# waldstein94/Stratified-Transformer

Hardware: AMD Instinct MI355X
Metric: points/sec through StratifiedAttention fwd+bwd, 100k-pt scene (higher is better)
Workload: dtype f32

## Files before the change

### include/pointops2_hip.h

```cpp
#ifndef POINTOPS2_HIP_H
#define POINTOPS2_HIP_H

#include <stddef.h>
#include <stdint.h>

#ifdef __cplusplus
extern "C" {
#endif

void pointops2_set_stream(void *hip_stream);
void *pointops2_get_stream(void);
const char *pointops2_last_error(void);
int pointops2_abi_version(void);
void pointops2_diag_set_fps_patience(unsigned long long ticks_100mhz);


void furthestsampling_cuda_launcher(int b, int n, const float *xyz, const int *offset,
                                    const int *new_offset, float *tmp, int *idx);

void knnquery_cuda_launcher(int m, int nsample, const float *xyz, const float *new_xyz,
                            const int *offset, const int *new_offset, int *idx, float *dist2);

void grouping_forward_cuda_launcher(int m, int nsample, int c, const float *input, const int *idx, float *output);
void grouping_backward_cuda_launcher(int m, int nsample, int c, const float *grad_output, const int *idx, float *grad_input);
// ... 144 lines not shown
    int n_pairs;
    int n_keyslots;
    const int *counts;
    const int *parent_first;
    const int *cell_perm;
    const int *cell_qstart;
    const int *cell_kbase;
    const int *cell_pbase;
    const int *cell_order;
    const int *qcell;
    const int *cell_keys;
    const int *kcell;
    const unsigned int *relp;
    int task_first;
    int task_step;
    int table_rows;
    int max_queries;
    const int *task_list;
    const int *task_count;
} pointops2_cell_plan;
size_t pointops2_cell_plan_workspace_bytes(int N);
void pointops2_cell_plan_count_launcher(int N, int max_queries, const int *s_cluster, const int *s_starts, const int *l_cluster,
                                        const int *ls_starts, int *cell_order, int *qcell, int *cell_desc, int *cell_qstart,
                                        int *cell_kbase, int *cell_pbase, int *cell_perm, int *parent_first, int *counts, void *ws,
                                        size_t ws_bytes);
void pointops2_cell_plan_prepare_launcher(int N, int max_queries, const int *s_cluster, const int *l_cluster, int *cell_order,
                                          int *parent_first, int *counts, void *ws, size_t ws_bytes);
void pointops2_cell_plan_sizes_launcher(int N, const int *s_cluster, const int *s_starts, const int *l_cluster, const int *ls_starts,
                                        const int *cell_order, int *qcell, int *cell_desc, int *cell_qstart, int *cell_kbase,
                                        int *cell_pbase, int *cell_perm, int *counts, void *ws, size_t ws_bytes);
void pointops2_cell_plan_fill_launcher(int N, const float *xyz, float window, float quant, int L, const int *s_order, const int *ls,
                                       const float *wc, const int *cell_order, const int *qcell, const int *cell_qstart,
                                       const int *cell_desc, const int *cell_kbase, const int *cell_pbase, int *cell_keys, int *kcell,
                                       unsigned int *relp);
void pointops2_swin_quant_launcher(int N, const float *xyz, const float *bbox6, float window, float quant, int shifted, int *q);
void pointops2_swin_pairs_rel_launcher(int N, int M, const int *index_0, const int *index_1, const int *q, int qgl, int *rel_idx);
void pointops2_swin_cell_fill_launcher(int N, int L, int qgl, const int *q, const int *s_order, const int *ls, const float *wc,
                                       const int *cell_order, const int *qcell, const int *cell_qstart, const int *cell_desc,
                                       const int *cell_kbase, const int *cell_pbase, int *cell_keys, int *kcell, unsigned int *relp);
void cell_attention_forward_launcher(const pointops2_cell_plan *plan, int h, int hdim, int L, const float *q, const float *k,
                                     const float *v, const float *table_q, const float *table_k, const float *table_v, float *out,
                                     float *ml, float *pbuf);
void cell_attention_backward_launcher(const pointops2_cell_plan *plan, int h, int hdim, int L, const float *grad_out, const float *q,
                                      const float *k, const float *v, const float *out, const float *table_q, const float *table_k,
                                      const float *table_v, const float *pbuf, float *gsbuf, float *grad_q, float *grad_k,
                                      float *grad_v, float *grad_table_q, float *grad_table_k, float *grad_table_v);
#define POINTOPS2_CELL_FWD_ERROR   (-1)
#define POINTOPS2_CELL_FWD_NONE    0
#define POINTOPS2_CELL_FWD_MFMA64  1
#define POINTOPS2_CELL_FWD_MFMA80  2
#define POINTOPS2_CELL_FWD_VALU80  3
#define POINTOPS2_CELL_FWD_VALU160 4
int pointops2_cell_forward_variant(const pointops2_cell_plan *plan, int h, int hdim, int L, int bf16);

void pointops2_voxel_keys_launcher(int N, int is_f64, const void *coord, double voxel, unsigned long long *keys);
void pointops2_crop_dist_launcher(int N, int is_f64, const void *coord, int seed, void *dist);

void cell_attention_forward_bf16_launcher(const pointops2_cell_plan *plan, int h, int hdim, int L, const uint16_t *q, const uint16_t *k,
                                          const uint16_t *v, const uint16_t *table_q, const uint16_t *table_k, const uint16_t *table_v,
                                          float *out, float *ml, float *pbuf);
void cell_attention_backward_bf16_launcher(const pointops2_cell_plan *plan, int h, int hdim, int L, const float *grad_out, const uint16_t *q,
                                           const uint16_t *k, const uint16_t *v, const float *out, const uint16_t *table_q,
                                           const uint16_t *table_k, const uint16_t *table_v, const float *pbuf, float *gsbuf, float *grad_q,
                                           float *grad_k, float *grad_v, float *grad_table_q, float *grad_table_k, float *grad_table_v);
#define POINTOPS2_ROWS_F32  0
#define POINTOPS2_ROWS_F16  1
#define POINTOPS2_ROWS_BF16 2
void cell_attention_qkv_forward_launcher(const pointops2_cell_plan *plan, int h, int hdim, int L, const void *qkv, int row_type, float scale,
                                         const float *table_q, const float *table_k, const float *table_v, float *out, float *ml, float *pbuf);
void cell_attention_qkv_backward_launcher(const pointops2_cell_plan *plan, int h, int hdim, int L, const float *grad_out, const void *qkv, int row_type,
                                          float scale, const float *out, const float *table_q, const float *table_k, const float *table_v,
                                          const float *pbuf, float *gsbuf, float *grad_qkv, float *grad_table_q, float *grad_table_k,
                                          float *grad_table_v);

void kpconv_aggregate_forward_launcher(int n_q, int n_s, int n_nb, int c, int n_kp, const float *query_xyz, const float *support_xyz,
                                       const int *neighbors, const float *feat, const float *k_points, float extent, float *wf);
void kpconv_aggregate_backward_launcher(int n_q, int n_s, int n_nb, int c, int n_kp, const float *query_xyz, const float *support_xyz,
                                        const int *neighbors, const float *k_points, float extent, const float *grad_wf,
                                        float *grad_feat);

void grouped_max_forward_launcher(int m, int n_s, int k, int c, int row_type, const void *feat, const int *idx, void *out,
                                  unsigned char *arg);
void grouped_max_backward_launcher(int m, int n_s, int k, int c, int row_type, const void *grad_out, const unsigned char *arg,
                                   const int *src_offsets, const int *src_pair, void *grad_feat);

void residual_norm_forward_launcher(int n, int c, int y_type, int o_type, const float *x, const void *y, const float *s, const float *gamma,
                                    const float *beta, float eps, float *z, void *o, float *stat);
void residual_norm_backward_launcher(int n, int c, int y_type, int o_type, const void *grad_o, const float *grad_z, const float *z,
                                     const float *stat, const float *s, const float *gamma, float *grad_x, void *grad_y, float *partials,
                                     int partial_rows, float *grad_gamma, float *grad_beta);

#define POINTOPS2_ACT_NONE       0
#define POINTOPS2_ACT_RELU       1
#define POINTOPS2_ACT_LEAKY_RELU 2
#define POINTOPS2_ACT_TANH       3
void batch_norm_act_stats_launcher(int n, int c, int x_type, const void *x, float *partials, int partial_rows, float eps, float momentum,
                                   float *running_mean, float *running_var, float *stat);
void batch_norm_act_forward_launcher(int n, int c, int x_type, int r_type, int act, float slope, const void *x, const float *mean,
                                     const float *scale, int scale_is_var, float eps, const float *gamma, const float *beta,
                                     const void *residual, void *o, float *stat_out);
void batch_norm_act_backward_launcher(int n, int c, int x_type, int act, float slope, int training, const void *x, const void *grad_o,
                                      const float *stat, const float *gamma, const float *beta, float *partials, int partial_rows,
                                      float *grad_gamma, float *grad_beta, void *grad_x);

void seg_loss_forward_launcher(int n, int c, int logits_type, int shift_type, const void *logits, const long long *target, const void *shift_pred,
                               const float *shift, long long ignore_index, float smooth_eps, float offset_weight, float *stat, double *partials,
// ... 69 lines not shown
```

### stratified_transformer_amd/_lib.py

```python
import ctypes
import os
import subprocess

import torch

_HERE = os.path.dirname(os.path.abspath(__file__))
LIB_PATH = os.path.join(_HERE, "lib", "libpointops2_hip.so")
CSRC = os.path.join(_HERE, "csrc")
_lib = None

I, U, P, Z, F, D = ctypes.c_int, ctypes.c_uint, ctypes.c_void_p, ctypes.c_size_t, ctypes.c_float, ctypes.c_double
Q = ctypes.c_longlong


class LaunchOpts(ctypes.Structure):
    _fields_ = [("table_rows", I), ("key_rows", I), ("csc_offsets", P), ("csc_pair", P), ("csc_query", P), ("row_order", P),
                ("row_order_rows", I), ("workspace", P), ("workspace_bytes", Z), ("point_count", I), ("batch_count", I),
                ("fps_prev_idx", P), ("fps_prev_new_offset", P), ("fps_unordered", I)]


def with_table_rows(opts, L):
    opts = opts if opts is not None else LaunchOpts()
    opts.table_rows = int(L)
    return opts
# ... 53 lines not shown
    "pointops2_cell_plan_sizes_launcher": [I, P, P, P, P, P, P, P, P, P, P, P, P, P, Z],
    "pointops2_cell_plan_fill_launcher": [I, P, F, F, I, P, P, P, P, P, P, P, P, P, P, P, P],
    "pointops2_swin_quant_launcher": [I, P, P, F, F, I, P],
    "pointops2_swin_pairs_rel_launcher": [I, I, P, P, P, I, P],
    "pointops2_swin_cell_fill_launcher": [I, I, I] + [P] * 13,
    "cell_attention_forward_launcher": [P, I, I, I] + [P] * 9,
    "cell_attention_backward_launcher": [P, I, I, I] + [P] * 16,
    "cell_attention_forward_bf16_launcher": [P, I, I, I] + [P] * 9,
    "cell_attention_backward_bf16_launcher": [P, I, I, I] + [P] * 16,
    "cell_attention_qkv_forward_launcher": [P, I, I, I, P, I, F] + [P] * 6,
    "cell_attention_qkv_backward_launcher": [P, I, I, I, P, P, I, F] + [P] * 10,
    "kpconv_aggregate_forward_launcher": [I, I, I, I, I, P, P, P, P, P, F, P],
    "kpconv_aggregate_backward_launcher": [I, I, I, I, I, P, P, P, P, F, P, P],
    "grouped_max_forward_launcher": [I, I, I, I, I, P, P, P, P],
    "grouped_max_backward_launcher": [I, I, I, I, I, P, P, P, P, P],
    "residual_norm_forward_launcher": [I, I, I, I, P, P, P, P, P, F, P, P, P],
    "residual_norm_backward_launcher": [I, I, I, I, P, P, P, P, P, P, P, P, P, I, P, P],
    "batch_norm_act_stats_launcher": [I, I, I, P, P, I, F, F, P, P, P],
    "batch_norm_act_forward_launcher": [I, I, I, I, I, F, P, P, P, I, F, P, P, P, P, P],
    "batch_norm_act_backward_launcher": [I, I, I, I, F, I, P, P, P, P, P, P, I, P, P, P],
    "seg_loss_forward_launcher": [I, I, I, I, P, P, P, P, Q, F, F, P, P, I, P, P, P],
    "seg_loss_backward_launcher": [I, I, I, I, P, P, P, P, P, P, P, Q, F, F, P, P],
    "pointops2_dbscan_keys_launcher": [I, I, P, P, D, D, D, D, I, I, I, P],
    "pointops2_dbscan_prepare_launcher": [I, I, I, I, I, P, P, P, P, P, P],
    "pointops2_dbscan_core_launcher": [I, I, P, P, P, P, P, P, P, P],
    "pointops2_dbscan_round_launcher": [I, I, P, P, P, P, P, P, P],
    "pointops2_dbscan_label_launcher": [I, I, P, P, P, P, P, P, P, P],
    "pointops2_contacts_count_launcher": [I, I, P, P, P, F, P, P],
    "pointops2_contacts_min_launcher": [I, I, P, P],
    "pointops2_label_boxes_launcher": [I, I, P, P, P, P, P],
    "pointops2_reach_rows_launcher": [I, I, P, P, P, F, P],
    "pointops2_supports_keys_launcher": [I, I, P, P, P, D, I, I, I, P],
    "pointops2_supports_means_launcher": [I, I, I, P, P, P, P, P, P, P, P],
    "pointops2_supports_count_launcher": [I, P, P, F, I, P],
    "pointops2_evaltile_seed_dist_launcher": [I, I, P, P, P, P, P, P],
    "pointops2_evaltile_update_launcher": [I, I, I, P, P, P, P, P],
    "pointops2_evaltile_vote_launcher": [I, I, I, I, P, P, P, P, P],
    "pointops2_evaltile_vote_shift_launcher": [I, I, I, I, P, I, P, P, P, P, P, P],
    "pointops2_augment_pass_launcher": [I] * 6 + [P] * 10,
    "pointops2_augment_blur_launcher": [Q, I, I, P, P, P],
}
RESULTS = {
    "pointops2_get_stream": ([], P),
    "pointops2_last_error": ([], ctypes.c_char_p),
    "pointops2_abi_version": ([], I),
    "pointops2_csc_workspace_bytes": ([I, I], Z),
    "pointops2_fps_workspace_bytes": ([I, I], Z),
    "pointops2_knn_workspace_bytes": ([I, I, I], Z),
    "pointops2_index_workspace_bytes": ([I], Z),
    "pointops2_partitions4_workspace_bytes": ([I], Z),
    "pointops2_row_order_workspace_bytes": ([I], Z),
    "pointops2_cell_plan_workspace_bytes": ([I], Z),
    "pointops2_cell_forward_variant": ([P, I, I, I, I], I),
    "pointops2_evaltile_max_parts": ([], I),
}

CELL_FWD = {"error": -1, "none": 0, "mfma64": 1, "mfma80": 2, "valu80": 3, "valu160": 4}
ROW_TYPES = {torch.float32: 0, torch.float16: 1, torch.bfloat16: 2}
ACTIVATIONS = {"none": 0, "relu": 1, "leaky_relu": 2, "tanh": 3}


def cell_forward_variant(plan, h, L, bf16=False, hdim=16):
    arg = None if plan is None else plan.c_arg() if hasattr(plan, "c_arg") else ctypes.byref(plan)
    code = lib().pointops2_cell_forward_variant(arg, int(h), int(hdim), int(L), int(bool(bf16)))
    return {v: k for k, v in CELL_FWD.items()}[code]


def exported_symbols():
    return sorted(list(SIGNATURES) + list(RESULTS))


def build(verbose=False):
    cmd = ["make", "-C", CSRC, "-j8"] + ([] if verbose else ["-s"])
    subprocess.check_call(cmd)
    return LIB_PATH


def lib():
    global _lib
    if _lib is None:
        if not os.path.exists(LIB_PATH):
            raise RuntimeError(
                f"{LIB_PATH} is missing: the HIP extension has not been built "
                "(run `python -c 'import __graft_entry__ as g; g.build()'` or `make -C stratified_transformer_amd/csrc`). "
                "There is no CPU fallback for the product path.")
        l = ctypes.CDLL(LIB_PATH)
        for name, argtypes in SIGNATURES.items():
            fn = getattr(l, name)
            fn.argtypes = argtypes
            fn.restype = None
        for name, (argtypes, restype) in RESULTS.items():
            fn = getattr(l, name)
            fn.argtypes = argtypes
            fn.restype = restype
        _lib = l
    return _lib


def ptr(t):
    if t is None:
        return None
    return t.data_ptr()


def check_tensor(t, dtype, name):
    if not t.is_cuda:
        raise RuntimeError(f"{name}: expected a GPU tensor (the pointops2 HIP path has no CPU fallback), got {t.device}")
    if t.dtype != dtype:
        raise TypeError(f"{name}: expected {dtype}, got {t.dtype}")
    if not t.is_contiguous():
        raise RuntimeError(f"{name}: expected a contiguous tensor")
    return t


_raw_stream = getattr(torch._C, "_cuda_getCurrentRawStream", None)


CALLS = [0]
# ... 17 lines not shown
```

### stratified_transformer_amd/csrc/cell_attn.hip

```cpp
#include "cell_common.h"

namespace p2 {


template <typename T>
__device__ __forceinline__ void stage_table_t(T *lds, const T *__restrict__ tab, int L, int h, int head) {
    const int total = 3 * L * 16;
    for (int x = threadIdx.x; x < total; x += blockDim.x) {
        const int i = x % 16, r = (x / 16) % L, ax = x / (16 * L);
        lds[x] = tab[(((size_t)r * h + head) * 16 + i) * 3 + ax];
    }
}
template <int TS, typename T>
__device__ __forceinline__ void stage_tables(T *lds, const T *__restrict__ table_q, const T *__restrict__ table_k, const T *__restrict__ table_v, int L,
                                             int h, int head) {
    stage_table_t<T>(lds, table_q, L, h, head);
    stage_table_t<T>(lds + TS, table_k, L, h, head);
    stage_table_t<T>(lds + 2 * TS, table_v, L, h, head);
    __syncthreads();
}

template <int LCAP>
struct TabGeo {
    static constexpr int TS = 3 * LCAP * 16;
// ... 3 lines not shown
    int o0, o1, o2;
};
__device__ __forceinline__ RowOff row_off(unsigned w, int L, int c) {
    RowOff r;
    r.o0 = (int)(w & 255u) * 16 + 4 * c;
    r.o1 = (int)(L + ((w >> 8) & 255u)) * 16 + 4 * c;
    r.o2 = (int)(2 * L + ((w >> 16) & 255u)) * 16 + 4 * c;
    return r;
}
template <int OFF>
__device__ __forceinline__ float4 tsum_at(const float *lds, RowOff r) {
    return add4(add4(*reinterpret_cast<const float4 *>(lds + OFF + r.o0), *reinterpret_cast<const float4 *>(lds + OFF + r.o1)),
                *reinterpret_cast<const float4 *>(lds + OFF + r.o2));
}

struct Rows3 {
    float4 a, b, c;
};
template <int OFF, typename T>
__device__ __forceinline__ Rows3 rows_at(const T *lds, RowOff r) {
    Rows3 x;
    x.a = ld_row4(lds + OFF + r.o0);
    x.b = ld_row4(lds + OFF + r.o1);
    x.c = ld_row4(lds + OFF + r.o2);
    return x;
}
typedef float f32x2c __attribute__((ext_vector_type(2)));
__device__ __forceinline__ float4 padd4(float4 a, float4 b) {
    const f32x2c lo = f32x2c{a.x, a.y} + f32x2c{b.x, b.y}, hi = f32x2c{a.z, a.w} + f32x2c{b.z, b.w};
    return make_float4(lo.x, lo.y, hi.x, hi.y);
}
__device__ __forceinline__ float4 pfma4(float s, float4 a, float4 acc) {
    const f32x2c ss = f32x2c{s, s};
    const f32x2c lo = __builtin_elementwise_fma(ss, f32x2c{a.x, a.y}, f32x2c{acc.x, acc.y});
    const f32x2c hi = __builtin_elementwise_fma(ss, f32x2c{a.z, a.w}, f32x2c{acc.z, acc.w});
    return make_float4(lo.x, lo.y, hi.x, hi.y);
}
__device__ __forceinline__ float4 rsum(Rows3 r) { return padd4(padd4(r.a, r.b), r.c); }
__device__ __forceinline__ f32x2c pdot_acc(float4 a, float4 b, f32x2c acc) {
    acc = __builtin_elementwise_fma(f32x2c{a.x, a.y}, f32x2c{b.x, b.y}, acc);
    return __builtin_elementwise_fma(f32x2c{a.z, a.w}, f32x2c{b.z, b.w}, acc);
}
__device__ __forceinline__ float pdot4(float4 a, float4 b) {
    const f32x2c r = pdot_acc(a, b, f32x2c{0.f, 0.f});
    return r.x + r.y;
}

template <int NPMAX, typename F>
__device__ __forceinline__ void dispatch_passes(int np, F f) {
    if (np <= 2) f(std::integral_constant<int, 2>{});
    else if (np == 3) f(std::integral_constant<int, 3>{});
    else if (np == 4 || NPMAX <= 4) f(std::integral_constant<int, 4>{});
    else if constexpr (NPMAX > 4) {
        if (np <= 6) f(std::integral_constant<int, 6>{});
        else f(std::integral_constant<int, 8>{});
    }
}

template <typename TT, bool PK>
struct LaneCtx {
    const TT *lds;
    int L, lane, p, c, head, h, C, hoff, rs_packed;
    float qscale;
    __device__ __forceinline__ int rs() const { return PK ? rs_packed : C; }
    template <typename RT>
    __device__ __forceinline__ float4 q_row4(const RT *q, int i) const {
        if constexpr (PK) return scaled_row4<RT>(q + (size_t)i * rs_packed + hoff, qscale);
        else return ld_row4(q + (size_t)i * C + hoff);
    }
};
template <typename TT, bool PK>
__device__ __forceinline__ LaneCtx<TT, PK> make_lane_ctx(const TT *lds, int h, int L, int rs, float qscale) {
    LaneCtx<TT, PK> x;
    x.lds = lds;
    x.L = L;
    x.h = h;
    x.head = blockIdx.y;
    x.C = h * 16;
    x.rs_packed = rs;
    x.qscale = qscale;
    x.lane = threadIdx.x & 63;
    x.p = x.lane >> 2;
    x.c = x.lane & 3;
    x.hoff = x.head * 16 + 4 * x.c;
    return x;
}

__device__ __forceinline__ void wait_vmem() {
    asm volatile("" ::: "memory");
    __builtin_amdgcn_s_waitcnt(0x0F70);
}
__device__ __forceinline__ int next_query_ids(rsrc_t qid, int off) {
    const int ids = (int)bload_u32(qid, off);
    wait_vmem();
    return ids;
}

template <int NPA, typename RT, typename T, bool PK>
__device__ __forceinline__ void load_key_rows(const LaneCtx<T, PK> &x, const CellBufs &cb, const RT *__restrict__ rows, int j0, int nvalid,
                                              float4 (&r4)[NPA]) {
    unsigned keys[NPA];
    bload_words<NPA>(cb.key, (j0 + x.p * NPA) * 4, keys);
#pragma unroll
    for (int t = 0; t < NPA; t++) {
        const float4 r = ld_row4(rows + (size_t)keys[t] * x.rs() + x.hoff);
        r4[t] = t < nvalid ? r : make_float4(0.f, 0.f, 0.f, 0.f);
    }
}
// ... 220 lines not shown
        wait_vmem();
        const int roff = (il * ct.nk + j0 + p * NPA) * 4;
        const float4 go4 = go_nx, o4 = o_nx;
        unsigned w[NPA];
        float a[NPA];
#pragma unroll
        for (int t = 0; t < NPA; t++) {
            w[t] = w_nx[t];
            a[t] = t < nvalid ? a_nx[t] : 0.f;
        }
        if (((il + 1) & 63) == 0) ids = next_query_ids(cb.qid, (il + 1 + x.lane) * 4);
        i_nx = __builtin_amdgcn_readlane(ids, (il + 1) & 63);
        go_nx = ldg4(go + (size_t)i_nx * x.C + x.hoff);
        o_nx = ldg4(out + (size_t)i_nx * x.C + x.hoff);
        bload_words<NPA>(cb.rel, roff + ct.nk * 4, w_nx);
        bload_floats<NPA>(rs_p, roff + ct.nk * 4, a_nx);
        if (il && c == 0) bstore_floats<NPA>(rs_g, roff - ct.nk * 4, gs_pv, nvalid);
        const float delta = quad_sum(pdot4(go4, o4));
        Rows3 rv = rows_at<2 * TS, T>(x.lds, row_off(w[0], x.L, c));
#pragma unroll
        for (int t = 0; t < NPA; t++) {
            Rows3 rv1 = rv;
            if (t + 1 < NPA) rv1 = rows_at<2 * TS, T>(x.lds, row_off(w[t + 1], x.L, c));
            const float ga = quad_sum(pdot4(go4, padd4(rsum(rv), v4[t])));
            gs_pv[t] = a[t] * (ga - delta);
            dv4[t] = pfma4(a[t], go4, dv4[t]);
            rv = rv1;
            __builtin_amdgcn_sched_barrier(0);
        }
    }
    if (ct.nq > 0 && c == 0) bstore_floats<NPA>(rs_g, ((ct.nq - 1) * ct.nk + j0 + p * NPA) * 4, gs_pv, nvalid);
    flush_key_grads<NPA, T, PK>(scr, dv4, cb.key, j0, nkc, grad_v, x);
}

template <int NPA, int TS, typename RT, typename T, bool PK>
__device__ __forceinline__ void bwd_sweep_keys(const LaneCtx<T, PK> &x, const CellTask &ct, const CellBufs &cb, rsrc_t rs_g, float *scr,
                                               const RT *__restrict__ q, const RT *__restrict__ k, float *__restrict__ grad_q,
                                               float *__restrict__ grad_k, int ch, int j0, int nkc) {
    const int p = x.p, c = x.c;
    const int nvalid = min(max(nkc - p * NPA, 0), NPA);
    float4 k4[NPA], dk4[NPA];
    load_key_rows<NPA, RT, T, PK>(x, cb, k, j0, nvalid, k4);
#pragma unroll
    for (int t = 0; t < NPA; t++) dk4[t] = make_float4(0.f, 0.f, 0.f, 0.f);
    unsigned w_nx[NPA];
    float g_nx[NPA];
    bload_words<NPA>(cb.rel, (j0 + p * NPA) * 4, w_nx);
    bload_floats<NPA>(rs_g, (j0 + p * NPA) * 4, g_nx);
    int ids = (int)bload_u32(cb.qid, x.lane * 4);
    int i_nx = __builtin_amdgcn_readlane(ids, 0);
    float4 q_nx = x.q_row4(q, i_nx);
    float4 tot_pv = make_float4(0.f, 0.f, 0.f, 0.f);
    int i_pv = 0;
    auto store_dq = [&](int i, float4 tot) {
        float *o = grad_q + (size_t)i * x.rs() + x.hoff;
        stg4(o, ch ? add4(tot, ldg4(o)) : tot);
    };
#pragma unroll 1
    for (int il = 0; il < ct.nq; il++) {
        wait_vmem();
        const int i = i_nx;
        const int roff = (il * ct.nk + j0 + p * NPA) * 4;
        const float4 q4 = q_nx;
        unsigned w[NPA];
        float g[NPA];
#pragma unroll
        for (int t = 0; t < NPA; t++) {
            w[t] = w_nx[t];
            g[t] = t < nvalid ? g_nx[t] : 0.f;
        }
        if (((il + 1) & 63) == 0) ids = next_query_ids(cb.qid, (il + 1 + x.lane) * 4);
        i_nx = __builtin_amdgcn_readlane(ids, (il + 1) & 63);
        q_nx = x.q_row4(q, i_nx);
        bload_words<NPA>(cb.rel, roff + ct.nk * 4, w_nx);
        bload_floats<NPA>(rs_g, roff + ct.nk * 4, g_nx);
        if (il && p == 0) store_dq(i_pv, tot_pv);
        float4 dq = make_float4(0.f, 0.f, 0.f, 0.f);
        RowOff ro = row_off(w[0], x.L, c);
        Rows3 rq = rows_at<0, T>(x.lds, ro), rk = rows_at<TS, T>(x.lds, ro);
#pragma unroll
        for (int t = 0; t < NPA; t++) {
            Rows3 rq1 = rq, rk1 = rk;
            if (t + 1 < NPA) {
                ro = row_off(w[t + 1], x.L, c);
                rq1 = rows_at<0, T>(x.lds, ro);
                rk1 = rows_at<TS, T>(x.lds, ro);
            }
            dq = pfma4(g[t], padd4(rsum(rq), k4[t]), dq);
            dk4[t] = pfma4(g[t], padd4(rsum(rk), q4), dk4[t]);
            rq = rq1;
            rk = rk1;
            __builtin_amdgcn_sched_barrier(0);
        }
        float4 tot = slots_sum16_4(dq);
        if constexpr (PK) tot = make_float4(tot.x * x.qscale, tot.y * x.qscale, tot.z * x.qscale, tot.w * x.qscale);
        tot_pv = tot;
        i_pv = i;
    }
    if (ct.nq > 0 && p == 0) store_dq(i_pv, tot_pv);
    flush_key_grads<NPA, T, PK>(scr, dk4, cb.key, j0, nkc, grad_k, x);
}

template <int NP, int LCAP, typename RT, typename T, bool PK>
__global__ __launch_bounds__(CA_WAVES_BWD * 64) void cell_bwd_kernel(pointops2_cell_plan pl, int h, int L, const float *__restrict__ go,
                                                                 const RT *__restrict__ q, const RT *__restrict__ k,
                                                                 const RT *__restrict__ v, int rs, float qscale, const float *__restrict__ out,
                                                                 const T *__restrict__ table_q, const T *__restrict__ table_k,
                                                                 const T *__restrict__ table_v, const float *__restrict__ pbuf,
                                                                 float *__restrict__ gsbuf, size_t plane, float *__restrict__ grad_q,
                                                                 float *__restrict__ grad_k, float *__restrict__ grad_v) {
    constexpr int TS = TabGeo<LCAP>::TS;
    extern __shared__ float lds_raw[];
    T *lds = reinterpret_cast<T *>(lds_raw);
    const LaneCtx<T, PK> x = make_lane_ctx<T, PK>(lds, h, L, rs, qscale);
    const int wave = __builtin_amdgcn_readfirstlane(threadIdx.x >> 6);
    float *scr = reinterpret_cast<float *>(lds + 3 * TS) + wave * 256;
    stage_tables<TS, T>(lds, table_q, table_k, table_v, L, h, x.head);
    const int nC = share_count(pl, pl.counts[0]);
    const float *pb = pbuf + (size_t)x.head * plane;
    float *gb = gsbuf + (size_t)x.head * plane;
    const int slots = gridDim.x * CA_WAVES_BWD, slot = blockIdx.x * CA_WAVES_BWD + wave;
    for (int round = 0; round * slots < nC; round++) {
        const int task = snake_task(round, slot, slots);
        if (task >= nC) continue;
        const CellTask ct = cell_task(pl, share_task(pl, task));
        const int nch = (ct.nk + 16 * NP - 1) / (16 * NP);
        const CellBufs cb = make_cell_bufs(pl, ct);
        const rsrc_t rs_p = tile_rsrc(pb, ct), rs_g = tile_rsrc(gb, ct);
        for (int ch = 0; ch < nch; ch++) {
            const int j0 = ch * 16 * NP, nkc = min(16 * NP, ct.nk - j0);
            dispatch_passes<NP>((nkc + 15) >> 4, [&](auto tag) {
                bwd_sweep_values<decltype(tag)::value, TS, RT, T, PK>(x, ct, cb, rs_p, rs_g, scr, go, out, v, grad_v, j0, nkc);
            });
        }
        for (int ch = 0; ch < nch; ch++) {
            const int j0 = ch * 16 * NP, nkc = min(16 * NP, ct.nk - j0);
            dispatch_passes<NP>((nkc + 15) >> 4, [&](auto tag) {
                bwd_sweep_keys<decltype(tag)::value, TS, RT, T, PK>(x, ct, cb, rs_g, scr, q, k, grad_q, grad_k, ch, j0, nkc);
            });
        }
    }
}

struct CFixScale {
    float mul, inv;
};
__device__ __forceinline__ CFixScale c_row_scale(unsigned maxbits, int n) {
    CFixScale sc;
    if (maxbits >= 0x7f800000u) {
        sc.mul = 0.f;
        sc.inv = __uint_as_float(0x7fc00000u);
        return sc;
    }
    const int E = (int)(maxbits >> 23) - 126;
    const int bits_n = 32 - __clz(max(n, 1));
    const int S = max(-126, min(126, 30 - bits_n - E));
    sc.mul = __uint_as_float((unsigned)(S + 127) << 23);
    sc.inv = __uint_as_float((unsigned)(127 - S) << 23);
    return sc;
}

constexpr int CT_WAVES = 8;

template <int TA>
struct CellTableGeo {
    static constexpr int LP = TA * 16;
    static constexpr int ROW = 3 * LP + 16;
    static constexpr size_t walk_bytes() { return (size_t)CT_WAVES * 4 * ROW * 4; }
    static constexpr size_t sum_bytes() { return (size_t)LP * 48 * 4; }
    static constexpr size_t lds_bytes() { return walk_bytes() > sum_bytes() ? walk_bytes() : sum_bytes(); }
};

template <int TA, bool BYKEY, bool SC, typename XT>
__device__ __forceinline__ void cell_table_grad_body(const pointops2_cell_plan &pl, int h, int L, const float *__restrict__ wbuf, size_t plane,
// ... 149 lines not shown

static const char *cell_refusal(const pointops2_cell_plan *plan, int hdim, int L, bool backward) {
    if (hdim != 16) return "cell_attention: d != 16";
    if (backward && (L < 1 || L > 80)) return "cell_attention backward: table rows L must be in 1..80";
    if (L < 1) return "cell_attention: no table rows";
    if (L != plan->table_rows)
        return backward ? "cell_attention backward: the tables' row count differs from the plan's table_rows"
                        : "cell_attention: the tables' row count differs from the plan's table_rows";
    if (L > 160) return "cell_attention: more than 160 table rows (use the operators)";
    return nullptr;
}

static int cell_fwd_variant(const pointops2_cell_plan *plan, int h, int hdim, int L, bool bf16, const char **why) {
    *why = nullptr;
    if (plan == nullptr || plan->n_points <= 0) return POINTOPS2_CELL_FWD_NONE;
    if ((*why = cell_refusal(plan, hdim, L, false)) != nullptr) return POINTOPS2_CELL_FWD_ERROR;
    if (L > 80) return POINTOPS2_CELL_FWD_VALU160;
    if (!bf16) {
        const double avg_queries = (double)plan->n_pairs / (double)(plan->n_keyslots > 0 ? plan->n_keyslots : 1);
        if (!((long long)plan->n_points * h >= 96000 && avg_queries < 15.0)) return L <= 64 ? POINTOPS2_CELL_FWD_MFMA64 : POINTOPS2_CELL_FWD_MFMA80;
    }
    return POINTOPS2_CELL_FWD_VALU80;
}

template <int LCAP, typename RT, typename TT, bool PK>
static void launch_valu_fwd(hipStream_t st, const pointops2_cell_plan *plan, int h, int L, const CellRows<RT> &r, const CellTables<TT> &t, float *out, float *ml,
                            float *pbuf) {
    const size_t lds = TabGeo<LCAP>::bytes(sizeof(TT));
    allow_big_lds(cell_fwd_kernel<CA_NP, LCAP, RT, TT, PK>, lds);
    const dim3 grid(cell_grid_x(1, plan->n_cells, h, CA_WAVES), h);
    hipLaunchKernelGGL((cell_fwd_kernel<CA_NP, LCAP, RT, TT, PK>), grid, dim3(CA_WAVES * 64), lds, st, *plan, h, L, r.q, r.k, r.v, r.rs, r.scale, t.q, t.k, t.v, out,
                       ml, pbuf, (size_t)plan->n_pairs);
}

template <typename RT, typename TT, bool PK>
static void launch_cell_fwd(hipStream_t st, const pointops2_cell_plan *plan, int h, int hdim, int L, const CellRows<RT> &r, const CellTables<TT> &t, float *out,
                            float *ml, float *pbuf) {
    const char *why;
    const int variant = cell_fwd_variant(plan, h, hdim, L, !std::is_same<TT, float>::value, &why);
    if (why != nullptr) { set_error(why); return; }
    if (variant == POINTOPS2_CELL_FWD_NONE) return;
    if constexpr (std::is_same<TT, float>::value) {
        if (variant == POINTOPS2_CELL_FWD_MFMA64 || variant == POINTOPS2_CELL_FWD_MFMA80) {
            cell_fwd_mfma_launch(st, variant, plan, h, L, RowTag<RT>::code, PK, CellRows<void>{r.q, r.k, r.v, r.rs, r.scale}, t, out, pbuf);
            check_launch();
            return;
        }
    }
    if (variant == POINTOPS2_CELL_FWD_VALU80) launch_valu_fwd<80, RT, TT, PK>(st, plan, h, L, r, t, out, ml, pbuf);
    else launch_valu_fwd<160, RT, TT, PK>(st, plan, h, L, r, t, out, ml, pbuf);
    check_launch();
}

template <typename RT, typename TT, bool PK>
static void launch_cell_bwd(hipStream_t st, const pointops2_cell_plan *plan, int h, int hdim, int L, const float *grad_out, const CellRows<RT> &r, const float *out,
                            const CellTables<TT> &t, const float *pbuf, float *gsbuf, const CellGrads &g, const CellGrads &gt) {
    if (plan == nullptr || plan->n_points <= 0) return;
    if (const char *why = cell_refusal(plan, hdim, L, true)) { set_error(why); return; }
    const size_t lds = TabGeo<80>::bytes(sizeof(TT)) + (size_t)CA_WAVES_BWD * 256 * sizeof(float);
    allow_big_lds(cell_bwd_kernel<CA_NP_BWD, 80, RT, TT, PK>, lds);
    const size_t plane = (size_t)plan->n_pairs;
    hipLaunchKernelGGL((cell_bwd_kernel<CA_NP_BWD, 80, RT, TT, PK>), dim3(cell_grid_x(1, plan->n_cells, h, CA_WAVES_BWD), h),
                       dim3(CA_WAVES_BWD * 64), lds, st, *plan, h, L, grad_out, r.q, r.k, r.v, r.rs, r.scale, out, t.q, t.k, t.v, pbuf, gsbuf, plane, g.q, g.k, g.v);
    const dim3 grid3(cell_grid_x(1, plan->n_cells, h, CT_WAVES), h, 3), tblock(CT_WAVES * 64);
    if (L <= 64) hipLaunchKernelGGL((cell_table_grad3_kernel<4, RT, PK>), grid3, tblock, CellTableGeo<4>::lds_bytes(), st, *plan, h, L, gsbuf, pbuf, plane, r.q, r.k,
                                    grad_out, gt.q, gt.k, gt.v, r.rs, r.scale);
    else hipLaunchKernelGGL((cell_table_grad3_kernel<5, RT, PK>), grid3, tblock, CellTableGeo<5>::lds_bytes(), st, *plan, h, L, gsbuf, pbuf, plane, r.q, r.k, grad_out,
                            gt.q, gt.k, gt.v, r.rs, r.scale);
    check_launch();
}

template <typename RT>
static CellRows<RT> packed_rows(const void *qkv, int h, float scale) {
    const RT *r = static_cast<const RT *>(qkv);
    return {r, r + h * 16, r + 2 * h * 16, 3 * h * 16, scale};
}

}

using namespace p2;

extern "C" {

int pointops2_cell_forward_variant(const pointops2_cell_plan *plan, int h, int hdim, int L, int bf16) {
    const char *why;
    return cell_fwd_variant(plan, h, hdim, L, bf16 != 0, &why);
}

void cell_attention_forward_launcher(const pointops2_cell_plan *plan, int h, int hdim, int L, const float *q, const float *k,
                                     const float *v, const float *table_q, const float *table_k, const float *table_v, float *out,
                                     float *ml, float *pbuf) {
    launch_cell_fwd<float, float, false>(begin_launch().stream, plan, h, hdim, L, {q, k, v, h * 16, 1.0f}, {table_q, table_k, table_v}, out, ml, pbuf);
}
void cell_attention_backward_launcher(const pointops2_cell_plan *plan, int h, int hdim, int L, const float *grad_out, const float *q,
                                      const float *k, const float *v, const float *out, const float *table_q, const float *table_k,
                                      const float *table_v, const float *pbuf, float *gsbuf, float *grad_q, float *grad_k,
                                      float *grad_v, float *grad_table_q, float *grad_table_k, float *grad_table_v) {
    launch_cell_bwd<float, float, false>(begin_launch().stream, plan, h, hdim, L, grad_out, {q, k, v, h * 16, 1.0f}, out, {table_q, table_k, table_v}, pbuf, gsbuf,
                                         {grad_q, grad_k, grad_v}, {grad_table_q, grad_table_k, grad_table_v});
}
void cell_attention_forward_bf16_launcher(const pointops2_cell_plan *plan, int h, int hdim, int L, const uint16_t *q, const uint16_t *k,
                                          const uint16_t *v, const uint16_t *table_q, const uint16_t *table_k, const uint16_t *table_v,
                                          float *out, float *ml, float *pbuf) {
    launch_cell_fwd<bf16_t, bf16_t, false>(begin_launch().stream, plan, h, hdim, L, {q, k, v, h * 16, 1.0f}, {table_q, table_k, table_v}, out, ml, pbuf);
}
void cell_attention_backward_bf16_launcher(const pointops2_cell_plan *plan, int h, int hdim, int L, const float *grad_out, const uint16_t *q,
                                           const uint16_t *k, const uint16_t *v, const float *out, const uint16_t *table_q,
                                           const uint16_t *table_k, const uint16_t *table_v, const float *pbuf, float *gsbuf, float *grad_q,
                                           float *grad_k, float *grad_v, float *grad_table_q, float *grad_table_k, float *grad_table_v) {
    launch_cell_bwd<bf16_t, bf16_t, false>(begin_launch().stream, plan, h, hdim, L, grad_out, {q, k, v, h * 16, 1.0f}, out, {table_q, table_k, table_v}, pbuf, gsbuf,
                                           {grad_q, grad_k, grad_v}, {grad_table_q, grad_table_k, grad_table_v});
}

void cell_attention_qkv_forward_launcher(const pointops2_cell_plan *plan, int h, int hdim, int L, const void *qkv, int row_type, float scale,
                                         const float *table_q, const float *table_k, const float *table_v, float *out, float *ml, float *pbuf) {
    const hipStream_t st = begin_launch().stream;
    if (!with_row_type(row_type, [&](auto tag) {
        using RT = typename decltype(tag)::type;
        launch_cell_fwd<RT, float, true>(st, plan, h, hdim, L, packed_rows<RT>(qkv, h, scale), {table_q, table_k, table_v}, out, ml, pbuf);
    })) set_error("cell_attention_qkv: unknown row_type");
}
void cell_attention_qkv_backward_launcher(const pointops2_cell_plan *plan, int h, int hdim, int L, const float *grad_out, const void *qkv, int row_type,
                                          float scale, const float *out, const float *table_q, const float *table_k, const float *table_v,
                                          const float *pbuf, float *gsbuf, float *grad_qkv, float *grad_table_q, float *grad_table_k,
                                          float *grad_table_v) {
    const hipStream_t st = begin_launch().stream;
    if (!with_row_type(row_type, [&](auto tag) {
        using RT = typename decltype(tag)::type;
        launch_cell_bwd<RT, float, true>(st, plan, h, hdim, L, grad_out, packed_rows<RT>(qkv, h, scale), out, {table_q, table_k, table_v}, pbuf, gsbuf,
                                         {grad_qkv, grad_qkv + h * 16, grad_qkv + 2 * h * 16}, {grad_table_q, grad_table_k, grad_table_v});
    })) set_error("cell_attention_qkv backward: unknown row_type");
}

}
```

### stratified_transformer_amd/csrc/cell_common.h

```cpp
#pragma once
#include "rpe_common.h"
#include "row_types.h"
#include <algorithm>

namespace p2 {

typedef float __attribute__((ext_vector_type(4))) f32x4c;

constexpr int CA_NP = 8;
constexpr int CA_NP_BWD = 3;
constexpr int CA_WAVES = 12;
constexpr int CA_WAVES_BWD = 12;

template <int CTRL>
__device__ __forceinline__ float dppf(float v) {
    return __int_as_float(__builtin_amdgcn_update_dpp(0, __float_as_int(v), CTRL, 0xF, 0xF, true));
}
__device__ __forceinline__ float swap16(float v) { return __int_as_float(__builtin_amdgcn_ds_swizzle(__float_as_int(v), 0x401F)); }
__device__ __forceinline__ float quad_sum(float v) {
    v += dppf<0xB1>(v);
    v += dppf<0x4E>(v);
    return v;
}
__device__ __forceinline__ float slots_sum16(float v) {
    v += dppf<0x124>(v);
    v += dppf<0x128>(v);
    v += swap16(v);
    v += __shfl_xor(v, 32, 64);
    return v;
}
__device__ __forceinline__ float slots_max16(float v) {
    v = fmaxf(v, dppf<0x124>(v));
    v = fmaxf(v, dppf<0x128>(v));
    v = fmaxf(v, swap16(v));
    v = fmaxf(v, __shfl_xor(v, 32, 64));
    return v;
}
__device__ __forceinline__ float4 slots_sum16_4(float4 v) {
    return make_float4(slots_sum16(v.x), slots_sum16(v.y), slots_sum16(v.z), slots_sum16(v.w));
}

template <typename RT>
__device__ __forceinline__ float4 scaled_row4(const RT *p, float scale) {
    const float4 r = ld_row4(p);
    return make_float4(round_rows<RT>(r.x * scale), round_rows<RT>(r.y * scale), round_rows<RT>(r.z * scale), round_rows<RT>(r.w * scale));
}
template <typename RT>
__device__ __forceinline__ float scaled_elem(const RT *p, float scale) { return round_rows<RT>(ld_elem(p) * scale); }

typedef __amdgpu_buffer_rsrc_t rsrc_t;
__device__ __forceinline__ rsrc_t make_rsrc(const void *base, unsigned bytes) {
    return __builtin_amdgcn_make_buffer_rsrc(const_cast<void *>(base), 0, (int)bytes, 0x00020000);
}
__device__ __forceinline__ unsigned bload_u32(rsrc_t r, int off) { return __builtin_amdgcn_raw_buffer_load_b32(r, off, 0, 0); }
__device__ __forceinline__ float bload_f32(rsrc_t r, int off) { return __uint_as_float(__builtin_amdgcn_raw_buffer_load_b32(r, off, 0, 0)); }
__device__ __forceinline__ void bstore_f32(rsrc_t r, int off, float v) { __builtin_amdgcn_raw_buffer_store_b32(__float_as_uint(v), r, off, 0, 0); }
typedef unsigned u32x2c __attribute__((ext_vector_type(2)));
typedef unsigned u32x3c __attribute__((ext_vector_type(3)));
typedef unsigned u32x4c __attribute__((ext_vector_type(4)));
template <int N>
__device__ __forceinline__ void bload_words(rsrc_t r, int off, unsigned (&w)[N]) {
    static_assert(N == 2 || N == 3 || N == 4 || N == 6 || N == 8, "pass counts of dispatch_passes");
    if constexpr (N == 2) {
        const u32x2c a = __builtin_amdgcn_raw_buffer_load_b64(r, off, 0, 0);
        w[0] = a.x; w[1] = a.y;
// ... 106 lines not shown
```

Before: 8.929 million.

## Add wide backward cell-attention variant selected by average keys per point

Adds a second backward kernel configuration (6 keys per lane, 8 waves) chosen when the average keys per point falls in a middle band, and templates the backward kernel on wave count. It also prefetches the old grad_q row one iteration early so the accumulate-store no longer waits on a fresh load. The wider variant aims to cover mid-sized cells with fewer passes over the key columns, at the cost of more registers per lane and fewer waves per block. A query function exposes which variant is picked.

```diff
diff --git a/include/pointops2_hip.h b/include/pointops2_hip.h
--- a/include/pointops2_hip.h
+++ b/include/pointops2_hip.h
@@ -220,6 +220,11 @@
 #define POINTOPS2_CELL_FWD_VALU80  3
 #define POINTOPS2_CELL_FWD_VALU160 4
 int pointops2_cell_forward_variant(const pointops2_cell_plan *plan, int h, int hdim, int L, int bf16);
+#define POINTOPS2_CELL_BWD_ERROR   (-1)
+#define POINTOPS2_CELL_BWD_NONE    0
+#define POINTOPS2_CELL_BWD_KEYS48  1
+#define POINTOPS2_CELL_BWD_KEYS96  2
+int pointops2_cell_backward_variant(const pointops2_cell_plan *plan, int h, int hdim, int L, int bf16);
 
 void pointops2_voxel_keys_launcher(int N, int is_f64, const void *coord, double voxel, unsigned long long *keys);
 void pointops2_crop_dist_launcher(int N, int is_f64, const void *coord, int seed, void *dist);
diff --git a/stratified_transformer_amd/_lib.py b/stratified_transformer_amd/_lib.py
--- a/stratified_transformer_amd/_lib.py
+++ b/stratified_transformer_amd/_lib.py
@@ -129,10 +129,12 @@
     "pointops2_row_order_workspace_bytes": ([I], Z),
     "pointops2_cell_plan_workspace_bytes": ([I], Z),
     "pointops2_cell_forward_variant": ([P, I, I, I, I], I),
+    "pointops2_cell_backward_variant": ([P, I, I, I, I], I),
     "pointops2_evaltile_max_parts": ([], I),
 }
 
 CELL_FWD = {"error": -1, "none": 0, "mfma64": 1, "mfma80": 2, "valu80": 3, "valu160": 4}
+CELL_BWD = {"error": -1, "none": 0, "keys48": 1, "keys96": 2}
 ROW_TYPES = {torch.float32: 0, torch.float16: 1, torch.bfloat16: 2}
 ACTIVATIONS = {"none": 0, "relu": 1, "leaky_relu": 2, "tanh": 3}
 
@@ -141,6 +143,12 @@
     arg = None if plan is None else plan.c_arg() if hasattr(plan, "c_arg") else ctypes.byref(plan)
     code = lib().pointops2_cell_forward_variant(arg, int(h), int(hdim), int(L), int(bool(bf16)))
     return {v: k for k, v in CELL_FWD.items()}[code]
+
+
+def cell_backward_variant(plan, h, L, bf16=False, hdim=16):
+    arg = None if plan is None else plan.c_arg() if hasattr(plan, "c_arg") else ctypes.byref(plan)
+    code = lib().pointops2_cell_backward_variant(arg, int(h), int(hdim), int(L), int(bool(bf16)))
+    return {v: k for k, v in CELL_BWD.items()}[code]
 
 
 def exported_symbols():
diff --git a/stratified_transformer_amd/csrc/cell_attn.hip b/stratified_transformer_amd/csrc/cell_attn.hip
--- a/stratified_transformer_amd/csrc/cell_attn.hip
+++ b/stratified_transformer_amd/csrc/cell_attn.hip
@@ -79,8 +79,8 @@
     else if (np == 3) f(std::integral_constant<int, 3>{});
     else if (np == 4 || NPMAX <= 4) f(std::integral_constant<int, 4>{});
     else if constexpr (NPMAX > 4) {
-        if (np <= 6) f(std::integral_constant<int, 6>{});
-        else f(std::integral_constant<int, 8>{});
+        if (np <= 6 || NPMAX <= 6) f(std::integral_constant<int, 6>{});
+        else if constexpr (NPMAX > 6) f(std::integral_constant<int, 8>{});
     }
 }
 
@@ -407,16 +407,14 @@
     float4 q_nx = x.q_row4(q, i_nx);
     float4 tot_pv = make_float4(0.f, 0.f, 0.f, 0.f);
     int i_pv = 0;
-    auto store_dq = [&](int i, float4 tot) {
-        float *o = grad_q + (size_t)i * x.rs() + x.hoff;
-        stg4(o, ch ? add4(tot, ldg4(o)) : tot);
-    };
+    float4 dq_old = make_float4(0.f, 0.f, 0.f, 0.f);
+    auto store_dq = [&](int i, float4 tot, float4 old) { stg4(grad_q + (size_t)i * x.rs() + x.hoff, ch ? add4(tot, old) : tot); };
 #pragma unroll 1
     for (int il = 0; il < ct.nq; il++) {
         wait_vmem();
         const int i = i_nx;
         const int roff = (il * ct.nk + j0 + p * NPA) * 4;
-        const float4 q4 = q_nx;
+        const float4 q4 = q_nx, dq_old_pv = dq_old;
         unsigned w[NPA];
         float g[NPA];
 #pragma unroll
@@ -429,7 +427,8 @@
         q_nx = x.q_row4(q, i_nx);
         bload_words<NPA>(cb.rel, roff + ct.nk * 4, w_nx);
         bload_floats<NPA>(rs_g, roff + ct.nk * 4, g_nx);
-        if (il && p == 0) store_dq(i_pv, tot_pv);
+        if (ch) dq_old = ldg4(grad_q + (size_t)i * x.rs() + x.hoff);
+        if (il && p == 0) store_dq(i_pv, tot_pv, dq_old_pv);
         float4 dq = make_float4(0.f, 0.f, 0.f, 0.f);
         RowOff ro = row_off(w[0], x.L, c);
         Rows3 rq = rows_at<0, T>(x.lds, ro), rk = rows_at<TS, T>(x.lds, ro);
@@ -452,12 +451,12 @@
         tot_pv = tot;
         i_pv = i;
     }
-    if (ct.nq > 0 && p == 0) store_dq(i_pv, tot_pv);
+    if (ct.nq > 0 && p == 0) store_dq(i_pv, tot_pv, dq_old);
     flush_key_grads<NPA, T, PK>(scr, dk4, cb.key, j0, nkc, grad_k, x);
 }
 
-template <int NP, int LCAP, typename RT, typename T, bool PK>
-__global__ __launch_bounds__(CA_WAVES_BWD * 64) void cell_bwd_kernel(pointops2_cell_plan pl, int h, int L, const float *__restrict__ go,
+template <int NP, int WAVES, int LCAP, typename RT, typename T, bool PK>
+__global__ __launch_bounds__(WAVES * 64) void cell_bwd_kernel(pointops2_cell_plan pl, int h, int L, const float *__restrict__ go,
                                                                  const RT *__restrict__ q, const RT *__restrict__ k,
                                                                  const RT *__restrict__ v, int rs, float qscale, const float *__restrict__ out,
                                                                  const T *__restrict__ table_q, const T *__restrict__ table_k,
@@ -474,7 +473,7 @@
     const int nC = share_count(pl, pl.counts[0]);
     const float *pb = pbuf + (size_t)x.head * plane;
     float *gb = gsbuf + (size_t)x.head * plane;
-    const int slots = gridDim.x * CA_WAVES_BWD, slot = blockIdx.x * CA_WAVES_BWD + wave;
+    const int slots = gridDim.x * WAVES, slot = blockIdx.x * WAVES + wave;
     for (int round = 0; round * slots < nC; round++) {
         const int task = snake_task(round, slot, slots);
         if (task >= nC) continue;
@@ -730,16 +729,36 @@
     check_launch();
 }
 
+constexpr double CELL_BWD_WIDE_MIN_KEYS = 51.0, CELL_BWD_WIDE_END_KEYS = 70.0;
+static int cell_bwd_variant(const pointops2_cell_plan *plan, int h, int hdim, int L, bool bf16, const char **why) {
+    *why = nullptr;
+    if (plan == nullptr || plan->n_points <= 0) return POINTOPS2_CELL_BWD_NONE;
+    if ((*why = cell_refusal(plan, hdim, L, true)) != nullptr) return POINTOPS2_CELL_BWD_ERROR;
+    (void)h;
+    (void)bf16;
+    const double avg_keys = (double)plan->n_pairs / (double)plan->n_points;
+    return avg_keys >= CELL_BWD_WIDE_MIN_KEYS && avg_keys < CELL_BWD_WIDE_END_KEYS ? POINTOPS2_CELL_BWD_KEYS96 : POINTOPS2_CELL_BWD_KEYS48;
+}
+
+template <int NP, int WAVES, typename RT, typename TT, bool PK>
+static void launch_bwd_sweeps(hipStream_t st, const pointops2_cell_plan *plan, int h, int L, const float *grad_out, const CellRows<RT> &r, const float *out,
+                              const CellTables<TT> &t, const float *pbuf, float *gsbuf, const CellGrads &g) {
+    const size_t lds = TabGeo<80>::bytes(sizeof(TT)) + (size_t)WAVES * 256 * sizeof(float);
+    allow_big_lds(cell_bwd_kernel<NP, WAVES, 80, RT, TT, PK>, lds);
+    hipLaunchKernelGGL((cell_bwd_kernel<NP, WAVES, 80, RT, TT, PK>), dim3(cell_grid_x(1, plan->n_cells, h, WAVES), h), dim3(WAVES * 64), lds, st, *plan, h, L,
+                       grad_out, r.q, r.k, r.v, r.rs, r.scale, out, t.q, t.k, t.v, pbuf, gsbuf, (size_t)plan->n_pairs, g.q, g.k, g.v);
+}
+
 template <typename RT, typename TT, bool PK>
 static void launch_cell_bwd(hipStream_t st, const pointops2_cell_plan *plan, int h, int hdim, int L, const float *grad_out, const CellRows<RT> &r, const float *out,
                             const CellTables<TT> &t, const float *pbuf, float *gsbuf, const CellGrads &g, const CellGrads &gt) {
-    if (plan == nullptr || plan->n_points <= 0) return;
-    if (const char *why = cell_refusal(plan, hdim, L, true)) { set_error(why); return; }
-    const size_t lds = TabGeo<80>::bytes(sizeof(TT)) + (size_t)CA_WAVES_BWD * 256 * sizeof(float);
-    allow_big_lds(cell_bwd_kernel<CA_NP_BWD, 80, RT, TT, PK>, lds);
+    const char *why;
+    const int variant = cell_bwd_variant(plan, h, hdim, L, !std::is_same<TT, float>::value, &why);
+    if (why != nullptr) { set_error(why); return; }
+    if (variant == POINTOPS2_CELL_BWD_NONE) return;
+    if (variant == POINTOPS2_CELL_BWD_KEYS96) launch_bwd_sweeps<CA_NP_BWD_WIDE, CA_WAVES_BWD_WIDE, RT, TT, PK>(st, plan, h, L, grad_out, r, out, t, pbuf, gsbuf, g);
+    else launch_bwd_sweeps<CA_NP_BWD, CA_WAVES_BWD, RT, TT, PK>(st, plan, h, L, grad_out, r, out, t, pbuf, gsbuf, g);
     const size_t plane = (size_t)plan->n_pairs;
-    hipLaunchKernelGGL((cell_bwd_kernel<CA_NP_BWD, 80, RT, TT, PK>), dim3(cell_grid_x(1, plan->n_cells, h, CA_WAVES_BWD), h),
-                       dim3(CA_WAVES_BWD * 64), lds, st, *plan, h, L, grad_out, r.q, r.k, r.v, r.rs, r.scale, out, t.q, t.k, t.v, pbuf, gsbuf, plane, g.q, g.k, g.v);
     const dim3 grid3(cell_grid_x(1, plan->n_cells, h, CT_WAVES), h, 3), tblock(CT_WAVES * 64);
     if (L <= 64) hipLaunchKernelGGL((cell_table_grad3_kernel<4, RT, PK>), grid3, tblock, CellTableGeo<4>::lds_bytes(), st, *plan, h, L, gsbuf, pbuf, plane, r.q, r.k,
                                     grad_out, gt.q, gt.k, gt.v, r.rs, r.scale);
@@ -763,6 +782,11 @@
 int pointops2_cell_forward_variant(const pointops2_cell_plan *plan, int h, int hdim, int L, int bf16) {
     const char *why;
     return cell_fwd_variant(plan, h, hdim, L, bf16 != 0, &why);
+}
+
+int pointops2_cell_backward_variant(const pointops2_cell_plan *plan, int h, int hdim, int L, int bf16) {
+    const char *why;
+    return cell_bwd_variant(plan, h, hdim, L, bf16 != 0, &why);
 }
 
 void cell_attention_forward_launcher(const pointops2_cell_plan *plan, int h, int hdim, int L, const float *q, const float *k,
diff --git a/stratified_transformer_amd/csrc/cell_common.h b/stratified_transformer_amd/csrc/cell_common.h
--- a/stratified_transformer_amd/csrc/cell_common.h
+++ b/stratified_transformer_amd/csrc/cell_common.h
@@ -11,6 +11,8 @@
 constexpr int CA_NP_BWD = 3;
 constexpr int CA_WAVES = 12;
 constexpr int CA_WAVES_BWD = 12;
+constexpr int CA_NP_BWD_WIDE = 6;
+constexpr int CA_WAVES_BWD_WIDE = 8;
 
 template <int CTRL>
 __device__ __forceinline__ float dppf(float v) {
```

Result: slower. 8.791 million (-1.6%).
